# hasindu2008/slow5tools

Measured on AMD Instinct MI355X. Metric: blow5_encode_raw_signal_throughput, higher is better.
Workload: dtype int16->u8

## Files before the change

### slow5tools_amd/csrc/deflate2_dev.h

```cpp
#pragma once

namespace s5 {

__device__ __forceinline__ uint32_t alignbit(uint32_t hi, uint32_t lo, uint32_t sh) { return __builtin_amdgcn_alignbit(hi, lo, sh); }
__device__ __forceinline__ uint32_t zbytes(uint32_t x) {
    const uint32_t t = (x & 0x7F7F7F7Fu) + 0x7F7F7F7Fu;
    return ~(t | x | 0x7F7F7F7Fu);
}
__device__ __forceinline__ uint32_t frame_mask(int a0, int first, int len) {
    const int lo = min(4, max(0, first - a0)), hi = min(4, max(0, len - a0));
    const uint32_t mh = hi >= 4 ? 0xFFFFFFFFu : (1u << (8 * hi)) - 1u;
    const uint32_t ml = lo >= 4 ? 0xFFFFFFFFu : (1u << (8 * lo)) - 1u;
    return mh & ~ml & 0x80808080u;
}
__device__ __forceinline__ int top_slot(uint32_t m) { return (31 - __clz((int)m)) >> 3; }

__device__ __forceinline__ void length_symbol(int L, uint32_t &sym, uint32_t &eb, uint32_t &ev) {
    const int l = L - 3;
    eb = 0; ev = 0;
    if (L == 258) sym = 285;
    else if (l < 8) sym = 257 + l;
    else {
        const int nb = 29 - __clz(l);
        sym = 261 + 4 * nb + ((l >> nb) & 3);
// ... 49 lines not shown
struct SlabTail {
    uint32_t ql;
    uint32_t nfull;
    uint32_t rem;
    uint32_t runbyte;
};
struct WaveCarry {
    int lastb;
    bool ok;
};
__device__ __forceinline__ SlabTail slab_tail(const uint8_t *__restrict__ buf, int k, const SlabCls &c, WaveCarry &wc) {
    const int lane = lane_id();
    const int p0 = 256 * k + 4 * lane - 2;
    const uint32_t lastmem = c.member & ~c.Cp1;
    const uint32_t Bm = c.V & ~c.C;
    const int lb = Bm ? p0 + top_slot(Bm) : -1;
    const int Lincl = wave_incl_max(lb);
    const int Lprev = (int)wave_prev((uint32_t)Lincl, 0xFFFFFFFFu);
    const int slab_last = __builtin_amdgcn_readlane(Lincl, 63);
    SlabTail t;
    t.ql = 4; t.nfull = 0; t.rem = 0; t.runbyte = 0;
    int s = 0;
    const bool has = lastmem != 0u;
    if (has) {
        t.ql = (uint32_t)top_slot(lastmem);
        const uint32_t below = Bm & ((1u << (8 * t.ql)) - 1u);
        s = below ? p0 + top_slot(below) : Lprev;
    }
    if (__ballot(has && s < 0)) {
        if (!wc.ok) { wc.lastb = find_break_before(buf, 256 * k - 2); wc.ok = true; }
        if (has && s < 0) s = wc.lastb;
    }
    if (slab_last >= 0) { wc.lastb = slab_last; wc.ok = true; }
    if (has) {
        const int body = p0 + (int)t.ql - s;
        t.nfull = (uint32_t)((body * 16257) >> 22);
        t.rem = (uint32_t)body - 258u * t.nfull;
        t.runbyte = (c.bytes >> (8 * t.ql)) & 255u;
    }
    return t;
}

__device__ __forceinline__ uint32_t length_extra_bits(uint32_t sym) { return sym >= 265u && sym < 285u ? (sym - 261u) >> 2 : 0u; }
__device__ __forceinline__ uint32_t carry_e_before(const uint32_t *__restrict__ buf32, int k, int len) {
    const int di = 64 * k - 1;
    const uint32_t w = buf32[di], wp = buf32[di - 1];
    return (uint32_t)__builtin_amdgcn_readfirstlane((int)(zbytes(w ^ alignbit(w, wp, 24)) & frame_mask(4 * di, 1, len)));
}

constexpr uint32_t DEFL2_LIST_CAP = 640;
constexpr uint32_t DEFL2_LISTB_MIN = 64;
constexpr uint32_t SEG_FAST = 0xFFFFFFFFu, SEG_REDO = 0xFFFFFFFEu, SEG_MASK = 0xFFFFFFFDu;

template <int TN = NT>
__device__ __forceinline__ void deflate2_prepare(DeflShared &S, uint32_t *obuf, uint32_t obuf_words) {
    constexpr int NWV = TN / 64;
    typedef uint32_t u4a __attribute__((ext_vector_type(4)));
    u4a *w16 = reinterpret_cast<u4a *>(obuf + (obuf_words - (uint32_t)(NWV * 288)));
    for (int i = threadIdx.x; i < NWV * 72; i += TN) w16[i] = u4a{0u, 0u, 0u, 0u};
    if (threadIdx.x == 0) { S.lalloc = 0; S.red[7] = 0; }
}

template <int MODE, int TN = NT>
__device__ __forceinline__ void deflate_block2(DeflShared &S, uint32_t *obuf, uint32_t obuf_words, const uint8_t *__restrict__ buf, int len,
                                               bool final, ZOut &z, uint32_t &adA, uint32_t &adB, uint32_t dbg = 0,
                                               EarlySize es = EarlySize{nullptr, 0}, uint32_t gen_hint = 0, bool prepared = false) {
    static_assert(MODE == 1 || MODE == 2, "fused single block (1) or staged multi-block (2): the bit buffer is this function's to clear");
    constexpr bool FUSED = MODE == 1;
    constexpr int NWV = TN / 64;
    static_assert(TN % 64 == 0 && NWV >= 4 && NWV <= 8, "S.wtot holds four words per wave");
    const int tid = threadIdx.x, lane = lane_id();
    const int wv = __builtin_amdgcn_readfirstlane(wave_id());
    if (len == 0) {
        for (uint32_t i = tid; i < obuf_words; i += TN) obuf[i] = 0;
        __syncthreads();
        if (tid == 0) { if (FUSED) put_bits(obuf, z, 64, 0x9c78u, 16); else obuf[0] = z.carry; }
        if (tid == 0) put_bits(obuf, z, z.bitpos, (final ? 1u : 0u) | (1u << 1), 10);
        z.bitpos += 10;
        publish_size(es, z.bitpos);
        __syncthreads();
        return;
    }
    const uint32_t wf_at = obuf_words - (uint32_t)(NWV * 288);
    uint32_t *wfa = obuf + wf_at;
    uint32_t *wf = wfa + wv * 288;
    if (!prepared) {
        deflate2_prepare<TN>(S, obuf, obuf_words);
        __syncthreads();
    }

    const uint32_t *buf32 = reinterpret_cast<const uint32_t *>(buf);
    constexpr bool POOLB = MODE == 2;
    const bool poolb_ok = POOLB && wf_at >= DEFL2_LISTB_MIN + 64u;
    uint16_t *tla = reinterpret_cast<uint16_t *>(S.freq);
    uint16_t *tlb_top = reinterpret_cast<uint16_t *>(obuf + wf_at);
    const uint32_t list_cap = DEFL2_LIST_CAP + (poolb_ok ? (wf_at - DEFL2_LISTB_MIN) * 2u : 0u);
    const int nsl = (len + 2 + 255) >> 8;
#ifndef S5_DEFL2_GEN_W
#define S5_DEFL2_GEN_W 4
#endif
#ifndef S5_DEFL2_GEN_W_FUSED
#define S5_DEFL2_GEN_W_FUSED 5
#endif
    constexpr int GW = FUSED ? S5_DEFL2_GEN_W_FUSED : S5_DEFL2_GEN_W;
    const int gs = min(nsl, gen_hint ? (int)((gen_hint + 2u + 255u) >> 8) : 0);
    const int cost_all = (GW - 1) * gs + nsl;
    auto bound = [&](int w) -> int {
        if (w >= NWV) return nsl;
        const int T = (cost_all * w + NWV / 2) / NWV;
        return T <= GW * gs ? (T + GW / 2) / GW : gs + (T - GW * gs);
    };
    const int k0 = bound(wv), k1 = bound(wv + 1);
    uint32_t segs = SEG_FAST;

    {
        uint32_t a_acc = 0, b_acc = 0, d_acc = 0, nmatch = 0, nextra = 0;
        uint32_t carryE = k0 > 0 && k0 < k1 ? carry_e_before(buf32, k0, len) : 0u;
        WaveCarry wc{-1, k0 == 0};
        for (int k = k0; k < k1; k++) {
#ifndef S5_DEFL2_NO_PAIRS
            if (k >= gs && k > 0 && k + 1 < k1 && 256 * k + 512 <= len) {
                const int d0 = 64 * k + 2 * lane;
                const uint32_t wp = buf32[d0 - 1], w0 = buf32[d0], w1 = buf32[d0 + 1];
                const uint32_t E0 = zbytes(w0 ^ alignbit(w0, wp, 24)), E1 = zbytes(w1 ^ alignbit(w1, w0, 24));
                const uint32_t EpA = dpp_u32<DPP_WAVE_SHR1>(carryE, E1);
                auto member_of = [](uint32_t E, uint32_t Ep) {
                    const uint32_t C = alignbit(E, Ep, 16), Cm1 = alignbit(E, Ep, 8), Cp1 = alignbit(E, Ep, 24);
                    return C & ((Cp1 & (E | Cm1)) | (Ep & Cm1));
                };
                if (__ballot((member_of(E0, EpA) | member_of(E1, E0)) != 0u) == 0ull) {
                    carryE = (uint32_t)__builtin_amdgcn_readlane((int)E1, 63);
                    const uint32_t bA = alignbit(w0, wp, 16), bB = alignbit(w1, w0, 16);
                    atomicAdd(&wf[bA & 255u], 1u);
                    atomicAdd(&wf[(bA >> 8) & 255u], 1u);
                    atomicAdd(&wf[(bA >> 16) & 255u], 1u);
                    atomicAdd(&wf[bA >> 24], 1u);
                    atomicAdd(&wf[bB & 255u], 1u);
                    atomicAdd(&wf[(bB >> 8) & 255u], 1u);
                    atomicAdd(&wf[(bB >> 16) & 255u], 1u);
                    atomicAdd(&wf[bB >> 24], 1u);
                    const uint32_t wA = (uint32_t)(len - (256 * k + 8 * lane - 2));
                    const uint32_t sA = __builtin_amdgcn_udot4(bA, 0x01010101u, 0u, false), sB = __builtin_amdgcn_udot4(bB, 0x01010101u, 0u, false);
                    a_acc += sA + sB;
                    b_acc = __umul24(wA, sA) + __umul24(wA - 4u, sB) + b_acc;
                    d_acc = __builtin_amdgcn_udot4(bA, 0x03020100u, d_acc, false);
                    d_acc = __builtin_amdgcn_udot4(bB, 0x03020100u, d_acc, false);
                    wc.ok = false;
                    k++;
                    continue;
                }
            }
#endif
            const bool full = k > 0 && 256 * k + 256 <= len;
            const uint32_t wgt = (uint32_t)(len - (256 * k + 4 * lane - 2));
            SlabCls c;
            if (full) c = classify_slab<false>(buf32, k, len, carryE);
            else c = classify_slab<true>(buf32, k, len, carryE);
            const bool anymem = __ballot(c.member != 0u) != 0ull;
            if (full && !anymem) {
                atomicAdd(&wf[c.bytes & 255u], 1u);
                atomicAdd(&wf[(c.bytes >> 8) & 255u], 1u);
                atomicAdd(&wf[(c.bytes >> 16) & 255u], 1u);
                atomicAdd(&wf[c.bytes >> 24], 1u);
                const uint32_t s4 = __builtin_amdgcn_udot4(c.bytes, 0x01010101u, 0u, false);
                a_acc += s4;
                b_acc = __umul24(wgt, s4) + b_acc;
                d_acc = __builtin_amdgcn_udot4(c.bytes, 0x03020100u, d_acc, false);
                wc.ok = false;
                continue;
            }
            {
                uint32_t bytes = c.bytes;
// ... 373 lines not shown
```

### slow5tools_amd/csrc/deflate_dev.h

```cpp
#pragma once
#include "dev_common.h"

namespace s5 {

constexpr int DEFL_BLK = NT * 64;
constexpr int NLIT = 286;
constexpr int DOFF = 288;

template <int CAP>
struct BuildScratchT {
    alignas(16) uint32_t lf[CAP];
    alignas(16) uint32_t nf[CAP];
    uint16_t npar[CAP];
    uint16_t rsym[CAP];
};
struct SortScratch {
    uint32_t bm[64 * 9];
    uint32_t cnt[64];
    uint32_t ovl[288];
};
struct BuildScratch : BuildScratchT<288> { SortScratch sort; };

struct DeflShared {
    alignas(16) uint32_t freq[320];
// ... 419 lines not shown
    {
        static constexpr uint32_t CLA[19] = {0x30001, 0x7002f, 0x7006f, 0x7001f, 0x7005f, 0x50003, 0x50013, 0x5000b, 0x5001b, 0x50007,
                                             0x30005, 0x20000, 0x20002, 0x7003f, 0x00000, 0x00000, 0x50017, 0x6000f, 0x7007f};
        static constexpr uint32_t CLB[19] = {0x30002, 0x60017, 0x7002f, 0x7006f, 0x60037, 0x5000b, 0x40005, 0x5001b, 0x50007, 0x4000d,
                                             0x30006, 0x30001, 0x20000, 0x7001f, 0x7005f, 0x7003f, 0x40003, 0x6000f, 0x7007f};
        const uint32_t ca = lane < 19 ? CLA[lane] : 0u, cb = lane < 19 ? CLB[lane] : 0u;
        const uint32_t f = lane < 19 ? S.clfreq[lane] : 0u;
        const uint32_t eb = lane == 16 ? 2u : lane == 17 ? 3u : lane == 18 ? 7u : 0u;
        const uint32_t costA = wave_sum(f * ((ca >> 16) + eb) + ((f && !(ca >> 16)) ? (1u << 24) : 0u));
        const uint32_t costB = wave_sum(f * ((cb >> 16) + eb));
        const bool useA = costA <= costB;
        if (lane < 19) { const uint32_t c = useA ? ca : cb; S.clcode[lane] = c; S.cllens[lane] = (uint8_t)(c >> 16); }
        if (lane == 0) { S.red[6] = useA ? costA : costB; S.hclen = useA ? 18u : 19u; }
    }
}

template <int TN = NT>
__device__ __forceinline__ void flush_words(uint32_t *obuf, uint32_t *out32, ZOut &z, bool final_all, uint32_t n_words = 0xFFFFFFFFu) {
    const int tid = threadIdx.x;
    const uint32_t full = final_all ? (z.bitpos + 31) >> 5 : z.bitpos >> 5;
    const uint32_t n = n_words != 0xFFFFFFFFu ? n_words : full - z.flushed;
    {
        typedef uint32_t u4u __attribute__((ext_vector_type(4), aligned(4)));
        typedef uint32_t u4a __attribute__((ext_vector_type(4)));
        const u4a *s16 = reinterpret_cast<const u4a *>(obuf);
        const uint32_t nv = n >> 2;
        for (uint32_t j = tid; j < nv; j += TN) {
            const uint32_t w = z.flushed + 4u * j;
            const u4a v = s16[j];
            if (w >= 2) *reinterpret_cast<u4u *>(out32 + w) = v;
            else { out32[w + 2] = v.z; out32[w + 3] = v.w; }
        }
        for (uint32_t i = 4u * nv + tid; i < n; i += TN) {
            const uint32_t w = z.flushed + i;
            if (w >= 2) out32[w] = obuf[i];
        }
    }
    if (final_all) return;
    __syncthreads();
    const uint32_t partial = obuf[n];
    __syncthreads();
    for (uint32_t i = tid; i <= n; i += TN) obuf[i] = i == 0 ? partial : 0u;
    __syncthreads();
    z.flushed = full;
}

}
#include "deflate2_dev.h"
namespace s5 {

template <typename M>
__device__ __forceinline__ uint32_t zlib_frame_fused(DeflShared &S, uint32_t *obuf, uint32_t obuf_words, const uint8_t *pay,
                                                     uint32_t plen, ZOut &z, uint32_t dbg = 0, EarlySize es = EarlySize{nullptr, 0}, uint32_t gen_hint = 0,
                                                     bool prepared = false) {
    const int tid = threadIdx.x;
    z.bitpos = 80;
    z.flushed = 0;
    uint32_t adA = 1, adB = 0;
    deflate_block2<1, NT>(S, obuf, obuf_words, pay, (int)plen, true, z, adA, adB, dbg, es, gen_hint, prepared);
    if (dbg) return 16;
    z.bitpos = (z.bitpos + 7) & ~7u;
    if (tid == 0 && plen) {
        uint32_t a = 0, b = 0;
        for (int w = 0; w < NW; w++) { a += S.wad[w]; b += S.wad[8 + w]; }
        adB = (uint32_t)(((uint64_t)plen + b) % 65521u);
        adA = (1u + a) % 65521u;
    }
    if (tid == 0) put_bits(obuf, z, z.bitpos, __builtin_bswap32((adB << 16) | adA), 32);
    z.bitpos += 32;
    __syncthreads();
    return z.bitpos >> 3;
}

template <typename M>
__device__ __forceinline__ uint32_t zlib_compress_fused(DeflShared &S, uint32_t *obuf, uint32_t obuf_words,
                                                        const uint8_t *pay, uint32_t plen, uint8_t *out, uint32_t dbg = 0, uint32_t gen_hint = 0, bool prepared = false) {
    ZOut z;
    const uint32_t total = zlib_frame_fused<M>(S, obuf, obuf_words, pay, plen, z, dbg, EarlySize{nullptr, 0}, gen_hint, prepared);
    if (dbg) {
        if (threadIdx.x == 0) *reinterpret_cast<uint32_t *>(out) = z.bitpos;
        if (dbg == 41 && threadIdx.x < 20) reinterpret_cast<uint32_t *>(out)[4 + threadIdx.x] = threadIdx.x < 19 ? S.clfreq[threadIdx.x] : S.red[6];
        return 16;
    }
    flush_words(obuf, reinterpret_cast<uint32_t *>(out), z, true);
    if (threadIdx.x == 0) *reinterpret_cast<uint64_t *>(out) = (uint64_t)(total - 8);
    return total;
}

constexpr uint64_t LB_MASK = (1ull << 62) - 1;
__device__ __forceinline__ uint64_t wave_sum64(uint64_t v) {
#pragma unroll
    for (int d = 32; d >= 1; d >>= 1) v += __shfl_xor(v, d);
    return v;
}
template <int E = 1>
__device__ __forceinline__ uint64_t lookback_offset(unsigned long long *st, uint32_t r, uint64_t mysize, uint32_t *err, bool published) {
    const int lane = lane_id();
    if (!published && lane == 0) __hip_atomic_store(&st[r], (1ull << 62) | mysize, __ATOMIC_RELAXED, __HIP_MEMORY_SCOPE_AGENT);
    uint64_t acc = 0;
    long long base = (long long)r - 1;
    uint32_t spins = 0;
    for (;;) {
        uint64_t v[E];
#pragma unroll
        for (int e = 0; e < E; e++) {
            const long long idx = base - 64 * e - lane;
            v[e] = idx >= 0 ? __hip_atomic_load(&st[idx], __ATOMIC_RELAXED, __HIP_MEMORY_SCOPE_AGENT) : (2ull << 62);
        }
        int outcome = 0;
#pragma unroll
        for (int e = 0; e < E; e++) {
            if (outcome) continue;
            const uint32_t f = (uint32_t)(v[e] >> 62);
            const uint64_t m0 = __ballot(f == 0), m2 = __ballot(f == 2);
            const int first0 = m0 ? __ffsll((long long)m0) - 1 : 64;
            const int first2 = m2 ? __ffsll((long long)m2) - 1 : 64;
            if (first2 < first0) {
                acc += lane <= first2 ? (v[e] & LB_MASK) : 0ull;
                outcome = 1;
            } else {
                acc += lane < first0 ? (v[e] & LB_MASK) : 0ull;
                if (first0 < 64) { base -= 64 * e + first0; outcome = 2; }
            }
        }
        if (outcome == 1) break;
        if (outcome == 0) { base -= 64 * E; continue; }
        if (++spins > (1u << 22)) { if (lane == 0) *err = 1; break; }
        __builtin_amdgcn_s_sleep(2);
    }
    const uint64_t excl = wave_sum64(acc);
    if (lane == 0) __hip_atomic_store(&st[r], (2ull << 62) | (excl + mysize), __ATOMIC_RELAXED, __HIP_MEMORY_SCOPE_AGENT);
// ... 16 lines not shown
```

### slow5tools_amd/csrc/kernels.hip

```cpp
#include <hip/hip_runtime.h>
#include <limits.h>
#include <stdint.h>
#include <stdio.h>
#include <stdlib.h>
#include <string.h>

#include <atomic>
#include <mutex>
#include <type_traits>
#include <vector>

#include "../../include/slow5gpu.h"
#include "deflate_dev.h"
#include "lz_dev.h"
#include "inflate_dev.h"
#include "inflate_simt_dev.h"
#include "inflate_par_dev.h"
#include "zstd_dev.h"
#include "zstd_enc_dev.h"
#include "svb_dev.h"
#include "exzd_dev.h"
#include "order_dev.h"
#include "event_dev.h"
#include "enc_plan.h"

using namespace s5;

extern "C" void s5gpu_set_error(const char *fmt, ...);
int s5host_set_option(const char *key, long value);
namespace fsk { int set_option(const char *key, long value); }
namespace dfk { int set_option(const char *key, long value); }
namespace dtwk { int path_set_option(const char *key, long value); }
namespace pilek { int set_option(const char *key, long value); }
extern uint32_t s5host_generation;
static_assert(s5plan::BLK == (uint32_t)DEFL_BLK && s5plan::SIG_SVB_ZD == S5GPU_SIG_SVB_ZD && s5plan::SIG_EX_ZD == S5GPU_SIG_EX_ZD, "enc_plan.h restates these");

#define HIP_TRY(x)                                                                                   \
    do {                                                                                             \
        hipError_t e_ = (x);                                                                         \
        if (e_ != hipSuccess) {                                                                      \
            s5gpu_set_error("%s failed: %s (%s:%d)", #x, hipGetErrorString(e_), __FILE__, __LINE__); \
            return S5GPU_ERR_HIP;                                                                    \
        }                                                                                            \
    } while (0)

extern __shared__ __attribute__((aligned(16))) uint8_t smem[];

constexpr uint32_t S_BYTES = (sizeof(DeflShared) + 15u) & ~15u;
constexpr uint32_t BZ_BYTES = (sizeof(BuildScratch) + 15u) & ~15u;
constexpr uint32_t B_BYTES = NW * 288u * 4u + 64u;
constexpr uint32_t OVF = 0xFFFFFFFFu;

struct EncParams {
    s5gpu_encode_args_t a;
    uint32_t obuf_words;
    uint32_t pay_cap;
    uint32_t dbg;
    uint32_t zseq;
    uint32_t tier = 0;
};

static uint32_t g_fused_tier2 = 0;
static uint32_t g_zstd_sequences = 1;

__device__ __forceinline__ uint32_t payload_bound_dev(const s5gpu_read_desc_t &d, int sig_method) {
    const uint32_t n = d.n_samples;
    const uint32_t sig = sig_method == S5GPU_SIG_SVB_ZD ? 4 + ((n + 3) >> 2) + 3 * n
                       : sig_method == S5GPU_SIG_EX_ZD ? 24 + 2 * (((n + 3) >> 2) + 4 * n) + n : 2 * n;
    return d.hdr_len + 8 + sig + d.aux_len;
}

template <bool EXZD = false>
__device__ __forceinline__ uint32_t build_payload(const s5gpu_encode_args_t &a, const s5gpu_read_desc_t &d,
                                                  uint8_t *pay, uint32_t cap, uint32_t *ws, uint32_t *red = nullptr) {
    const int tid = threadIdx.x;
    const uint32_t n = d.n_samples;
    if constexpr (EXZD) {
        const uint32_t fixed_x = d.hdr_len + 8 + d.aux_len;
        if (fixed_x + 16 > cap) return OVF;
        const uint8_t *hdr = a.hdr + d.hdr_off;
        for (uint32_t i = tid; i < d.hdr_len; i += NT) pay[i] = hdr[i];
        uint8_t *lenp = pay + d.hdr_len;
        const uint32_t blen = exzd_encode_wg(a.sig + d.sig_off, n, lenp + 8, ws, red, cap - fixed_x);
        if (blen == EXZD_ERR) return OVF;
        if (tid < 8) lenp[tid] = tid < 4 ? (uint8_t)(blen >> (8 * tid)) : 0;
        if (d.aux_len) {
            const uint8_t *aux = a.aux + d.aux_off;
            uint8_t *ap = lenp + 8 + blen;
            for (uint32_t i = tid; i < d.aux_len; i += NT) ap[i] = aux[i];
        }
        return d.hdr_len + 8 + blen + d.aux_len;
    } else {
    const bool svb = a.sig_method == S5GPU_SIG_SVB_ZD;
    const uint32_t nk = (n + 3) >> 2;
    const uint32_t fixed = d.hdr_len + 8 + (svb ? 4 + nk : 0) + d.aux_len;
    if (fixed > cap || (svb ? n : 2 * n) > cap - fixed) return OVF;
    const uint8_t *hdr = a.hdr + d.hdr_off;
    for (uint32_t i = tid; i < d.hdr_len; i += NT) pay[i] = hdr[i];
    uint8_t *lenp = pay + d.hdr_len;
    uint8_t *sigp = lenp + 8;
    const int16_t *sig = a.sig + d.sig_off;
    uint64_t L;
    uint32_t sig_bytes;
    if (svb) {
        uint8_t *keys = sigp + 4;
        uint8_t *data = keys + nk;
        uint32_t total = 0;
        const uint32_t room = cap - fixed;
        for (uint32_t t0 = 0; t0 < n; t0 += SVB_TILE) {
            const uint32_t t = svb_encode_tile(sig, n, t0, keys + (t0 >> 2), data + total, ws, room - total, true);
            if (t > room - total) return OVF;
            total += t;
        }
        L = 4ull + nk + total;
        sig_bytes = (uint32_t)L;
// ... 33 lines not shown
        const uint32_t t = svb_encode_tile(sig, n, t0, reinterpret_cast<uint8_t *>(tile_keys), reinterpret_cast<uint8_t *>(tile_data), ws, OVF - 1);
        __syncthreads();
        const uint32_t tk = (min(n - t0, (uint32_t)SVB_TILE) + 3) >> 2;
        copy_record_out(tile_keys, tk, keys + (t0 >> 2));
        copy_record_out(tile_data, t, data + total);
        total += t;
        __syncthreads();
    }
    const uint64_t L = 4ull + nk + total;
    if (tid < 4) sigp[tid] = (uint8_t)(n >> (8 * tid));
    if (tid < 8) lenp[tid] = (uint8_t)(L >> (8 * tid));
    if (d.aux_len) {
        const uint8_t *aux = a.aux + d.aux_off;
        uint8_t *ap = sigp + (uint32_t)L;
        for (uint32_t i = tid; i < d.aux_len; i += NT) ap[i] = aux[i];
    }
    return d.hdr_len + 8 + (uint32_t)L + d.aux_len;
}

__device__ __forceinline__ uint32_t run_heavy_front(const s5gpu_encode_args_t &a, const s5gpu_read_desc_t &d) {
    return a.sig_method == S5GPU_SIG_SVB_ZD ? d.hdr_len + 12u + ((d.n_samples + 3u) >> 2) : 0u;
}

#ifndef S5_FUSED_HINT
#define S5_FUSED_HINT(a, d) run_heavy_front(a, d)
#endif

#ifndef S5_FUSED_WG_PER_CU
#define S5_FUSED_WG_PER_CU 8
#endif
template <typename M, bool EXZD = false, int WPS = S5_FUSED_WG_PER_CU>
__global__ __launch_bounds__(NT, WPS) void k_encode_fused(EncParams p) {
    const uint32_t r = blockIdx.x;
    if (p.tier == 2 && p.a.out_len[r] != 0) return;
    DeflShared &S = *reinterpret_cast<DeflShared *>(smem);
    uint32_t *obuf = reinterpret_cast<uint32_t *>(smem + S_BYTES);
    uint8_t *pay = smem + S_BYTES + 4u * p.obuf_words;
    const s5gpu_read_desc_t d = p.a.desc[r];
    deflate2_prepare<NT>(S, obuf, p.obuf_words);
    const uint32_t plen = build_payload<EXZD>(p.a, d, pay, p.pay_cap, S.ws, S.red);
    if (plen == OVF) {
        if (threadIdx.x == 0 && p.tier != 1) {
            const uint32_t at = atomicAdd(&p.a.ovf[0], 1u);
            p.a.ovf[1 + at] = r;
        }
        return;
    }
    __syncthreads();
    if (p.dbg == 1) {
        if (threadIdx.x == 0) p.a.out_len[r] = plen + pay[plen - 1];
        return;
    }
    uint8_t *out = p.a.slots + d.out_off;
    const uint32_t total = zlib_compress_fused<M>(S, obuf, p.obuf_words, pay, plen, out, p.dbg, S5_FUSED_HINT(p.a, d), true);
    if (threadIdx.x == 0) p.a.out_len[r] = total;
}

#ifndef S5_LB_E
#define S5_LB_E 1
#endif
struct StreamParams {
    unsigned long long *state;
    uint32_t *ctl;
    uint8_t *stream;
    uint64_t *rec_off;
};
template <typename M, bool EXZD = false>
__global__ __launch_bounds__(NT, S5_FUSED_WG_PER_CU) void k_encode_stream(EncParams p, StreamParams sp) {
    __shared__ uint32_t s_r;
    __shared__ uint64_t s_off;
    DeflShared &S = *reinterpret_cast<DeflShared *>(smem);
    uint32_t *obuf = reinterpret_cast<uint32_t *>(smem + S_BYTES);
    uint8_t *pay = smem + S_BYTES + 4u * p.obuf_words;
#ifdef S5_ES_NOTICKET
    const uint32_t r = blockIdx.x;
#else
    if (threadIdx.x == 0) s_r = atomicAdd(&sp.ctl[1], 1u);
    __syncthreads();
    const uint32_t r = s_r;
#endif
    const s5gpu_read_desc_t d = p.a.desc[r];
    deflate2_prepare<NT>(S, obuf, p.obuf_words);
    const uint32_t plen = build_payload<EXZD>(p.a, d, pay, p.pay_cap, S.ws, S.red);
    uint32_t total = 0;
    if (plen == OVF) {
        if (threadIdx.x == 0) atomicAdd(&sp.ctl[0], 1u);
    } else {
        __syncthreads();
        ZOut z;
        total = zlib_frame_fused<M>(S, obuf, p.obuf_words, pay, plen, z, 0, EarlySize{sp.state, r}, S5_FUSED_HINT(p.a, d), true);
        if (threadIdx.x == 0) { obuf[0] = total - 8; obuf[1] = 0; }
    }
    if (wave_id() == 0) {
        const uint64_t off = lookback_offset<S5_LB_E>(sp.state, r, total, &sp.ctl[2], plen != OVF);
        if (lane_id() == 0) {
            s_off = off;
            sp.rec_off[r] = off;
            if (r == p.a.n_reads - 1) sp.rec_off[p.a.n_reads] = off + total;
            p.a.out_len[r] = total;
        }
    }
    __syncthreads();
    if (total) copy_record_out(obuf, total, sp.stream + s_off);
}

__device__ __forceinline__ uint32_t park_offset(const s5gpu_read_desc_t &d, int sig_method) {
    return (d.slot_cap - payload_bound_dev(d, sig_method)) & ~15u;
}

#ifndef S5_PACK_WG
#define S5_PACK_WG 8
#endif
__global__ __launch_bounds__(NT, S5_PACK_WG) void k_pack(EncParams p, int mode, const uint32_t *ord) {
    __shared__ uint32_t ws[16];
    __shared__ __attribute__((aligned(16))) uint32_t tile_keys[SVB_TILE / 16 + 4];
    __shared__ __attribute__((aligned(16))) uint32_t tile_data[3 * SVB_TILE / 4 + 4];
    const uint32_t count = mode == 2 ? p.a.ovf[0] : p.a.n_reads;
    for (uint32_t it = blockIdx.x; it < count; it += gridDim.x) {
        const uint32_t r = mode == 2 ? ovf_at(p.a.ovf, ord, it) : it;
        const s5gpu_read_desc_t d = p.a.desc[r];
        uint8_t *dst = p.a.slots + d.out_off + (mode == 1 ? 8u : park_offset(d, p.a.sig_method));
        const uint32_t plen = build_payload_hbm(p.a, d, dst, ws, tile_keys, tile_data);
        if (threadIdx.x == 0) {
            if (mode == 1) {
                *reinterpret_cast<uint64_t *>(p.a.slots + d.out_off) = plen;
                p.a.out_len[r] = plen + 8;
            } else {
                p.a.out_len[r] = plen;
            }
        }
        __syncthreads();
    }
}

#ifndef S5_STAGED_TN
#define S5_STAGED_TN 256
#endif
struct StagedPf { uint4 v[DEFL_BLK / 16 / S5_STAGED_TN]; };
__device__ __forceinline__ void staged_fetch(StagedPf &pf, const uint8_t *src, uint32_t at, uint32_t plen) {
    const uint32_t bl = min(plen - at, (uint32_t)DEFL_BLK);
    const uint4 *s4 = reinterpret_cast<const uint4 *>(src + at);
#pragma unroll
    for (int j = 0; j < DEFL_BLK / 16 / S5_STAGED_TN; j++) {
        const uint32_t i = threadIdx.x + j * S5_STAGED_TN;
        pf.v[j] = i < (bl + 15) / 16 ? s4[i] : uint4{0u, 0u, 0u, 0u};
    }
}
__device__ __forceinline__ uint32_t deflate_staged_record(const EncParams &p, uint32_t r, const s5gpu_read_desc_t &d, uint32_t plen, DeflShared &S, uint32_t *obuf, BuildScratch &B, uint8_t *stage,
                                                          StagedPf &pf, const uint8_t *next_src, uint32_t next_plen) {
    const int tid = threadIdx.x;
    uint8_t *out = p.a.slots + d.out_off;
    const uint8_t *src = out + park_offset(d, p.a.sig_method);
// ... 1180 lines not shown
template <class Key>
static int build_order(const Key &key, uint32_t n, bool list, uint32_t long_bucket, hipStream_t st, const uint32_t **out,
                       std::unique_lock<std::mutex> &hold, size_t extra_words = 0, uint32_t **extra = nullptr) {
    *out = nullptr;
    if (extra) *extra = nullptr;
    if (!list && !(extra && extra_words)) return S5GPU_OK;
    const size_t list_words = list ? (((size_t)ORD_LIST + n + 3) & ~(size_t)3) : 0;
    uint32_t *p = nullptr;
    { const int rc = order_scratch(st, list_words + (extra ? extra_words : 0), &p, hold); if (rc) return rc; }
    if (!p) return S5GPU_OK;
    if (list) {
        const uint32_t nb = (n + NT - 1) / NT;
        hipLaunchKernelGGL(k_order_zero, dim3(1), dim3(NT), 0, st, p);
        hipLaunchKernelGGL(k_order_count<Key>, dim3(nb), dim3(NT), 0, st, key, p);
        hipLaunchKernelGGL(k_order_scan, dim3(1), dim3(128), 0, st, p, long_bucket);
        hipLaunchKernelGGL(k_order_scatter<Key>, dim3(nb), dim3(NT), 0, st, key, p);
        *out = p;
    }
    if (extra && extra_words) *extra = p + list_words;
    return S5GPU_OK;
}
static int launch_order(const s5gpu_decode_args_t *a, hipStream_t st, const uint32_t **out, std::unique_lock<std::mutex> &hold,
                        size_t extra_words = 0, uint32_t **extra = nullptr, bool want_order = true) {
    const bool order = want_order && g_order_min && a->n_recs >= g_order_min;
    return build_order(OrderByInLen{a->desc, a->n_recs}, a->n_recs, order, 0, st, out, hold, extra_words, extra);
}
static uint32_t g_zstd_pre_min = 256;
static size_t zstd_pre_words(const s5gpu_decode_args_t *a) {
    return g_zstd_pre_min && a->n_recs >= g_zstd_pre_min ? (size_t)a->n_recs * (ZW_REC / 4) : 0;
}
static int launch_eorder(const s5gpu_encode_args_t *a, hipStream_t st, const uint32_t **out, std::unique_lock<std::mutex> &hold) {
    const bool order = g_order_min && a->n_reads >= g_order_min;
    return build_order(OrderOvfBySamples{a->desc, a->ovf}, a->n_reads, order, 0, st, out, hold);
}
int s5kern_digest_order(const digk::DigRecs &R, hipStream_t st, const uint32_t **out, std::unique_lock<std::mutex> &hold) {
    return build_order(OrderByCanonLen{R.desc, R.fields, R.n}, R.n, R.n > 16, 0, st, out, hold);
}
int s5kern_event_order(const sigk::SigRecs &R, hipStream_t st, const uint32_t **out, std::unique_lock<std::mutex> &hold) {
    return build_order(OrderBySigLen{R}, R.n, R.n > 64, 0, st, out, hold);
}

static bool rec_method_ok(int m) { return m == S5GPU_REC_NONE || m == S5GPU_REC_ZLIB || m == S5GPU_REC_ZSTD; }
static bool sig_method_ok(int m) { return m == S5GPU_SIG_NONE || m == S5GPU_SIG_SVB_ZD || m == S5GPU_SIG_EX_ZD; }
static int enc_check(const s5gpu_encode_args_t *a) {
    if (!a || (a->n_reads && (!a->desc || !a->sig || !a->hdr || !a->slots || !a->out_len))) return S5GPU_ERR_ARG;
    return rec_method_ok(a->rec_method) && sig_method_ok(a->sig_method) ? S5GPU_OK : S5GPU_ERR_ARG;
}

static EncParams enc_params(const s5gpu_encode_args_t *a, bool dbg = false) {
    EncParams p;
    p.a = *a;
    p.dbg = dbg && getenv("S5GPU_DEBUG_STAGE") ? (uint32_t)atoi(getenv("S5GPU_DEBUG_STAGE")) : 0;
    p.zseq = g_zstd_sequences;
    p.obuf_words = 0; p.pay_cap = 0;
    return p;
}
static size_t staged_shape(EncParams &p) {
    p.obuf_words = (DEFL_BLK + 64) / 4; p.pay_cap = DEFL_BLK;
    return S_BYTES + 4ull * p.obuf_words + DEFL_BLK;
}
static size_t fused_shape(EncParams &p, uint32_t cap, uint32_t floor) {
    p.obuf_words = (cap + 64 > floor ? cap + 64 : floor) / 4; p.pay_cap = cap;
    return S_BYTES + 4ull * p.obuf_words + cap;
}
static int stream_params(StreamParams *sp, uint32_t n_reads, uint8_t *stream_out, uint64_t *rec_off, uint64_t *state, uint32_t *ctl, hipStream_t st) {
    *sp = StreamParams{reinterpret_cast<unsigned long long *>(state), ctl, stream_out, rec_off};
    HIP_TRY(hipMemsetAsync(state, 0, 8ull * n_reads, st));
    HIP_TRY(hipMemsetAsync(ctl, 0, 16, st));
    return S5GPU_OK;
}

using EncodeKernel = void (*)(EncParams);
using StreamKernel = void (*)(EncParams, StreamParams);
static const EncodeKernel ENCODE_FUSED[] = {k_encode_fused<uint32_t, false>, k_encode_fused<uint32_t, true>, k_encode_fused<uint64_t, false>, k_encode_fused<uint64_t, true>,
                                            k_encode_fused<uint64_t, false, 4>};
static const StreamKernel ENCODE_STREAM[] = {k_encode_stream<uint32_t, false>, k_encode_stream<uint32_t, true>, k_encode_stream<uint64_t, false>, k_encode_stream<uint64_t, true>};
static const EncodeKernel ZSTD_FUSED[] = {k_zstd_fused<false>, k_zstd_fused<true>};
static EncodeKernel encode_fused_kernel(bool wide, bool exzd, bool four_per_cu = false) { return ENCODE_FUSED[four_per_cu ? 4 : 2 * wide + exzd]; }
static StreamKernel encode_stream_kernel(bool wide, bool exzd) { return ENCODE_STREAM[2 * wide + exzd]; }
static EncodeKernel zstd_fused_kernel(bool exzd) { return ZSTD_FUSED[exzd]; }
static const void *const LDS_KERNELS[] = {(const void *)k_deflate_staged, (const void *)k_deflate_lz<LzLong>, (const void *)k_deflate_lz<LzShort>, (const void *)k_zstd_staged,
                                          (const void *)k_svbzd_encode, (const void *)k_svbzd_stream, (const void *)k_inflate_simt<false>, (const void *)k_inflate_simt<true>};

constexpr int DEV_MAX = 64;
struct DeviceFacts {
    std::atomic<bool> attrs{false};
    std::atomic<int> cus{0};
    std::atomic<uint32_t> np_resident[6];
} static g_dev[DEV_MAX];
static DeviceFacts *device_facts() {
    int dev = -1;
    return hipGetDevice(&dev) == hipSuccess && dev >= 0 && dev < DEV_MAX ? &g_dev[dev] : nullptr;
}
static int device_cus(int *cus) {
    DeviceFacts *f = device_facts();
    *cus = f ? f->cus.load(std::memory_order_relaxed) : 0;
    if (*cus > 0) return S5GPU_OK;
    int dev = 0;
    HIP_TRY(hipGetDevice(&dev));
    HIP_TRY(hipDeviceGetAttribute(cus, hipDeviceAttributeMultiprocessorCount, dev));
    if (f && *cus > 0) f->cus.store(*cus, std::memory_order_relaxed);
    return S5GPU_OK;
}
static int set_lds_attrs() {
    DeviceFacts *f = device_facts();
    if (f && f->attrs.load(std::memory_order_acquire)) return S5GPU_OK;
// ... 94 lines not shown
        return S5GPU_ERR_ARG;
    }
    if (a->n_reads == 0) return S5GPU_OK;
    int rc;
    if ((rc = set_lds_attrs())) return rc;
    hipStream_t st = (hipStream_t)stream_;
    EncParams p = enc_params(a);
    StreamParams sp;
    if ((rc = stream_params(&sp, a->n_reads, stream_out, rec_off, state, ctl, st))) return rc;
    const uint32_t cap = s5plan::fused_cap(a->sig_method, a->max_payload, a->lds_payload_cap, DEFL_BLK);
    const size_t lds = fused_shape(p, cap, B_BYTES);
    hipLaunchKernelGGL(encode_stream_kernel(s5plan::wide(cap), a->sig_method == S5GPU_SIG_EX_ZD), dim3(a->n_reads), dim3(NT), lds, st, p, sp);
    HIP_TRY(hipGetLastError());
    return S5GPU_OK;
}

extern "C" int s5gpu_pack_parked_dev(const s5gpu_encode_args_t *a, void *stream_) {
    int rc = enc_check(a);
    if (rc) { s5gpu_set_error("s5gpu_pack_parked_dev: bad arguments"); return rc; }
    if (a->n_reads == 0) return S5GPU_OK;
    EncParams p = enc_params(a);
    staged_shape(p);
    hipLaunchKernelGGL(k_pack, dim3(a->n_reads), dim3(NT), 0, (hipStream_t)stream_, p, 0, nullptr);
    HIP_TRY(hipGetLastError());
    return S5GPU_OK;
}

extern "C" int s5gpu_deflate_parked_dev(const s5gpu_encode_args_t *a, void *stream_) {
    int rc = enc_check(a);
    if (rc) { s5gpu_set_error("s5gpu_deflate_parked_dev: bad arguments"); return rc; }
    if (a->n_reads == 0) return S5GPU_OK;
    if ((rc = set_lds_attrs())) return rc;
    EncParams p = enc_params(a);
    const size_t lds = staged_shape(p);
    if (a->rec_method == S5GPU_REC_ZSTD) hipLaunchKernelGGL(k_zstd_staged, dim3(a->n_reads), dim3(NT), lds, (hipStream_t)stream_, p, 0);
    else if (a->sig_method == S5GPU_SIG_NONE)
        launch_lz(p, a->n_reads, a->max_payload, (hipStream_t)stream_);
    else hipLaunchKernelGGL(k_deflate_staged, dim3(a->n_reads), dim3(S5_STAGED_TN), lds, (hipStream_t)stream_, p, 0, nullptr);
    HIP_TRY(hipGetLastError());
    return S5GPU_OK;
}

static uint32_t g_unpack_fused = 1;
static uint32_t g_inflate_par = 1;
static uint32_t g_inflate_route = 1;
static uint32_t g_np_lds_payload = 1;
static uint32_t g_inflate_simt_min = 24576;
static const struct Option { const char *name; uint32_t *var; long lo, hi; uint32_t keep; } OPTIONS[] = {
    {"inflate_simt_min", &g_inflate_simt_min, 0, LONG_MAX, ~0u},
    {"inflate_route", &g_inflate_route, 0, 1, ~0u},
    {"np_lds_payload", &g_np_lds_payload, 0, 1, ~0u},
    {"fused_tier2", &g_fused_tier2, 0, DEFL_BLK, ~15u},
    {"zstd_sequences", &g_zstd_sequences, 0, 1, ~0u},
    {"unpack_fused", &g_unpack_fused, 0, 1, ~0u},
    {"inflate_par", &g_inflate_par, 0, 2, ~0u},
    {"zstd_pre_min", &g_zstd_pre_min, 0, LONG_MAX, ~0u},
    {"order_min", &g_order_min, 0, LONG_MAX, ~0u},
};
extern "C" int s5gpu_set_option(const char *key, long value) {
    for (const Option &o : OPTIONS)
        if (key && strcmp(key, o.name) == 0 && value >= o.lo && value <= o.hi) { *o.var = (uint32_t)value & o.keep; return S5GPU_OK; }
    if (s5host_set_option(key, value) == S5GPU_OK || fsk::set_option(key, value) == S5GPU_OK || dfk::set_option(key, value) == S5GPU_OK ||
        dtwk::path_set_option(key, value) == S5GPU_OK || pilek::set_option(key, value) == S5GPU_OK)
        return S5GPU_OK;
    s5gpu_set_error("s5gpu_set_option: unknown option");
    return S5GPU_ERR_ARG;
}
struct AuxStream {
    hipStream_t st = nullptr;
    hipEvent_t fork = nullptr, join = nullptr;
    int dev = -1;
};
static std::mutex g_aux_mu;
static std::vector<AuxStream *> g_aux_all, g_aux_free;
static int aux_acquire(AuxStream **out) {
    int dev = 0;
    HIP_TRY(hipGetDevice(&dev));
    {
        std::lock_guard<std::mutex> lk(g_aux_mu);
        for (size_t i = 0; i < g_aux_free.size(); i++)
            if (g_aux_free[i]->dev == dev) { *out = g_aux_free[i]; g_aux_free.erase(g_aux_free.begin() + (long)i); return S5GPU_OK; }
    }
    AuxStream *a = new AuxStream();
    a->dev = dev;
    if (hipStreamCreateWithFlags(&a->st, hipStreamNonBlocking) != hipSuccess || hipEventCreateWithFlags(&a->fork, hipEventDisableTiming) != hipSuccess ||
        hipEventCreateWithFlags(&a->join, hipEventDisableTiming) != hipSuccess) {
        if (a->st) (void)hipStreamDestroy(a->st);
        if (a->fork) (void)hipEventDestroy(a->fork);
        delete a;
        s5gpu_set_error("helper stream for the routed inflate could not be created");
        return S5GPU_ERR_HIP;
    }
    std::lock_guard<std::mutex> lk(g_aux_mu);
    g_aux_all.push_back(a);
    *out = a;
    return S5GPU_OK;
}
static void aux_release(AuxStream *a, uint32_t gen) {
    std::lock_guard<std::mutex> lk(g_aux_mu);
    if (gen == s5host_generation) g_aux_free.push_back(a);
}
void s5kern_release_aux() {
    std::lock_guard<std::mutex> lk(g_aux_mu);
    for (AuxStream *a : g_aux_all) {
        (void)hipStreamDestroy(a->st);
        (void)hipEventDestroy(a->fork);
// ... 350 lines not shown
```

Baseline: 686.9.

## Add run-list front pass for the generated prefix of fused deflate blocks

Result: no change. 685.5 (-0.2%).

```diff
diff --git a/slow5tools_amd/csrc/deflate2_dev.h b/slow5tools_amd/csrc/deflate2_dev.h
--- a/slow5tools_amd/csrc/deflate2_dev.h
+++ b/slow5tools_amd/csrc/deflate2_dev.h
@@ -125,6 +125,107 @@
 constexpr uint32_t DEFL2_LISTB_MIN = 64;
 constexpr uint32_t SEG_FAST = 0xFFFFFFFFu, SEG_REDO = 0xFFFFFFFEu, SEG_MASK = 0xFFFFFFFDu;
 
+#ifndef S5_DEFL2_RUNS_PER_SLAB
+#define S5_DEFL2_RUNS_PER_SLAB 128
+#endif
+constexpr int DEFL2_RUNS_HW = S5_DEFL2_RUNS_PER_SLAB + 2;
+__device__ __forceinline__ bool front_runs(DeflShared &S, uint32_t *obuf, uint32_t *wf, const uint8_t *__restrict__ buf, int len, int ka, int kb,
+                                           uint32_t carryE, uint32_t &a_acc, uint32_t &b_acc, uint32_t &d_acc, uint32_t &nmatch, uint32_t &nextra,
+                                           uint32_t &segs) {
+    const int lane = lane_id();
+    const uint32_t *buf32 = reinterpret_cast<const uint32_t *>(buf);
+    const int R0 = ka ? 256 * ka - 2 : 0, R1 = 256 * kb - 2;
+    uint16_t *L = reinterpret_cast<uint16_t *>(obuf) + DEFL2_RUNS_HW * ka;
+    const uint32_t lcap = (uint32_t)(DEFL2_RUNS_HW * (kb - ka)) - 1u;
+    const int ent = ka > 0 ? __builtin_amdgcn_readfirstlane((int)(buf[R0] == buf[R0 - 1])) : 0;
+    int nbk = 0;
+    uint32_t aa = 0, bb = 0, dd = 0, ub = 0;
+    for (int k = ka; k < kb; k++) {
+        const bool full = k > 0 && 256 * k + 256 <= len;
+        SlabCls c;
+        if (full) c = classify_slab<false>(buf32, k, len, carryE);
+        else c = classify_slab<true>(buf32, k, len, carryE);
+        uint32_t bytes = c.bytes;
+        if (!full) { const uint32_t vb = c.V >> 7; bytes &= (vb << 8) - vb; }
+        const uint32_t s4 = __builtin_amdgcn_udot4(bytes, 0x01010101u, 0u, false);
+        aa += s4;
+        bb = __umul24((uint32_t)(len - (256 * k + 4 * lane - 2)), s4) + bb;
+        dd = __builtin_amdgcn_udot4(bytes, 0x03020100u, dd, false);
+        ub += (uint32_t)__popc(c.V & ~c.member) + 2u * (uint32_t)__popc(c.member & ~c.Cp1);
+        const uint32_t Bm = c.V & ~c.C;
+        const uint32_t pop = (uint32_t)__popc(Bm);
+        const uint32_t incl = wave_incl_add(pop);
+        uint32_t at = (uint32_t)(ent + nbk) + incl - pop;
+        const uint32_t p0 = (uint32_t)(256 * k + 4 * lane - 2);
+#pragma unroll
+        for (int q = 0; q < 4; q++)
+            if (Bm & (0x80u << (8 * q))) L[min(at++, lcap)] = (uint16_t)(p0 + q);
+        nbk += __builtin_amdgcn_readlane((int)incl, 63);
+    }
+    if (nbk > S5_DEFL2_RUNS_PER_SLAB * (kb - ka)) return false;
+    const int nr = nbk + ent;
+    int sE = R0;
+    {
+        const int p = R1 + lane;
+        const bool brk = lane >= 3 || p >= len || buf[p] != buf[p - 1];
+        const int qend = R1 + __ffsll((long long)__ballot(brk)) - 1;
+        if (ent) sE = find_break_before(buf, R0);
+        if (lane == 0) { L[nr] = (uint16_t)qend; if (ent) L[0] = (uint16_t)sE; }
+    }
+    wave_sync();
+    const uint32_t room = wave_sum(ub) + (uint32_t)(((R1 - sE) * 16257) >> 22);
+    uint32_t st = 0;
+    if (lane == 0) st = atomicAdd(&S.lalloc, room);
+    st = (uint32_t)__builtin_amdgcn_readfirstlane((int)st);
+    const bool listed = st + room <= DEFL2_LIST_CAP;
+    uint16_t *tl = reinterpret_cast<uint16_t *>(S.freq);
+    uint32_t base = st;
+    for (int j0 = 0; j0 < nr; j0 += 64) {
+        const int j = j0 + lane;
+        int s = 0;
+        uint32_t own = 0, nfull = 0, mlen = 0, nl = 0;
+        if (j < nr) {
+            s = L[j];
+            const int q = L[j + 1];
+            own = s >= R0 ? 1u : 0u;
+            const int body = q - s - 1;
+            if (body < 3) nl = (uint32_t)max(0, min(q, R1) - max(s + 1, R0));
+            else if (q <= R1) {
+                nfull = (uint32_t)((body * 16257) >> 22);
+                const uint32_t rem = (uint32_t)body - 258u * nfull;
+                if (rem >= 3u) mlen = rem; else nl = rem;
+            }
+        }
+        const uint32_t ext = nfull + (mlen ? 1u : nl), cnt = own + ext;
+        const uint32_t incl = wave_incl_add(cnt);
+        if (cnt) {
+            const uint32_t b = buf[s];
+            uint32_t at = base + incl - cnt;
+            uint32_t last = b;
+            if (own + nl) atomicAdd(&wf[b], own + nl);
+            if (nfull) atomicAdd(&wf[285], nfull);
+            if (mlen) {
+                uint32_t tsym, teb, tev;
+                length_symbol((int)mlen, tsym, teb, tev);
+                atomicAdd(&wf[tsym], 1u);
+                nextra += teb;
+                last = tsym | (tev << 9);
+            }
+            nmatch += nfull + (mlen ? 1u : 0u);
+            if (listed) {
+                if (own) tl[at] = (uint16_t)b;
+                at += own;
+#pragma unroll 1
+                for (uint32_t i = 0; i < ext; i++) tl[at + i] = (uint16_t)(i < nfull ? 285u : last);
+            }
+        }
+        base += (uint32_t)__builtin_amdgcn_readlane((int)incl, 63);
+    }
+    if (lane < kb - ka) segs = listed ? st | (lane == 0 ? (base - st) << 16 : 0u) : SEG_REDO;
+    a_acc += aa; b_acc += bb; d_acc += dd;
+    return true;
+}
+
 template <int TN = NT>
 __device__ __forceinline__ void deflate2_prepare(DeflShared &S, uint32_t *obuf, uint32_t obuf_words) {
     constexpr int NWV = TN / 64;
@@ -137,7 +238,8 @@
 template <int MODE, int TN = NT>
 __device__ __forceinline__ void deflate_block2(DeflShared &S, uint32_t *obuf, uint32_t obuf_words, const uint8_t *__restrict__ buf, int len,
                                                bool final, ZOut &z, uint32_t &adA, uint32_t &adB, uint32_t dbg = 0,
-                                               EarlySize es = EarlySize{nullptr, 0}, uint32_t gen_hint = 0, bool prepared = false) {
+                                               EarlySize es = EarlySize{nullptr, 0}, uint32_t gen_hint = 0, bool prepared = false,
+                                               bool front = true) {
     static_assert(MODE == 1 || MODE == 2, "fused single block (1) or staged multi-block (2): the bit buffer is this function's to clear");
     constexpr bool FUSED = MODE == 1;
     constexpr int NWV = TN / 64;
@@ -190,7 +292,16 @@
         uint32_t a_acc = 0, b_acc = 0, d_acc = 0, nmatch = 0, nextra = 0;
         uint32_t carryE = k0 > 0 && k0 < k1 ? carry_e_before(buf32, k0, len) : 0u;
         WaveCarry wc{-1, k0 == 0};
-        for (int k = k0; k < k1; k++) {
+        int kfirst = k0;
+        if (FUSED && front) {
+            const int kb = min(k1, (int)(min(gen_hint, (uint32_t)len) + 2u) >> 8);
+            if (kb > k0 && (uint32_t)(DEFL2_RUNS_HW * kb + 1) / 2u <= wf_at && front_runs(S, obuf, wf, buf, len, k0, kb, carryE, a_acc, b_acc, d_acc, nmatch, nextra, segs)) {
+                kfirst = kb;
+                if (kb < k1) carryE = carry_e_before(buf32, kb, len);
+                wc = WaveCarry{-1, false};
+            }
+        }
+        for (int k = kfirst; k < k1; k++) {
 #ifndef S5_DEFL2_NO_PAIRS
             if (k >= gs && k > 0 && k + 1 < k1 && 256 * k + 512 <= len) {
                 const int d0 = 64 * k + 2 * lane;
diff --git a/slow5tools_amd/csrc/deflate_dev.h b/slow5tools_amd/csrc/deflate_dev.h
--- a/slow5tools_amd/csrc/deflate_dev.h
+++ b/slow5tools_amd/csrc/deflate_dev.h
@@ -495,12 +495,12 @@
 template <typename M>
 __device__ __forceinline__ uint32_t zlib_frame_fused(DeflShared &S, uint32_t *obuf, uint32_t obuf_words, const uint8_t *pay,
                                                      uint32_t plen, ZOut &z, uint32_t dbg = 0, EarlySize es = EarlySize{nullptr, 0}, uint32_t gen_hint = 0,
-                                                     bool prepared = false) {
+                                                     bool prepared = false, bool front_runs = true) {
     const int tid = threadIdx.x;
     z.bitpos = 80;
     z.flushed = 0;
     uint32_t adA = 1, adB = 0;
-    deflate_block2<1, NT>(S, obuf, obuf_words, pay, (int)plen, true, z, adA, adB, dbg, es, gen_hint, prepared);
+    deflate_block2<1, NT>(S, obuf, obuf_words, pay, (int)plen, true, z, adA, adB, dbg, es, gen_hint, prepared, front_runs);
     if (dbg) return 16;
     z.bitpos = (z.bitpos + 7) & ~7u;
     if (tid == 0 && plen) {
@@ -517,9 +517,10 @@
 
 template <typename M>
 __device__ __forceinline__ uint32_t zlib_compress_fused(DeflShared &S, uint32_t *obuf, uint32_t obuf_words,
-                                                        const uint8_t *pay, uint32_t plen, uint8_t *out, uint32_t dbg = 0, uint32_t gen_hint = 0, bool prepared = false) {
+                                                        const uint8_t *pay, uint32_t plen, uint8_t *out, uint32_t dbg = 0, uint32_t gen_hint = 0, bool prepared = false,
+                                                        bool front_runs = true) {
     ZOut z;
-    const uint32_t total = zlib_frame_fused<M>(S, obuf, obuf_words, pay, plen, z, dbg, EarlySize{nullptr, 0}, gen_hint, prepared);
+    const uint32_t total = zlib_frame_fused<M>(S, obuf, obuf_words, pay, plen, z, dbg, EarlySize{nullptr, 0}, gen_hint, prepared, front_runs);
     if (dbg) {
         if (threadIdx.x == 0) *reinterpret_cast<uint32_t *>(out) = z.bitpos;
         if (dbg == 41 && threadIdx.x < 20) reinterpret_cast<uint32_t *>(out)[4 + threadIdx.x] = threadIdx.x < 19 ? S.clfreq[threadIdx.x] : S.red[6];
diff --git a/slow5tools_amd/csrc/kernels.hip b/slow5tools_amd/csrc/kernels.hip
--- a/slow5tools_amd/csrc/kernels.hip
+++ b/slow5tools_amd/csrc/kernels.hip
@@ -57,10 +57,12 @@
     uint32_t pay_cap;
     uint32_t dbg;
     uint32_t zseq;
+    uint32_t front_runs;
     uint32_t tier = 0;
 };
 
 static uint32_t g_fused_tier2 = 0;
+static uint32_t g_front_runs = 1;
 static uint32_t g_zstd_sequences = 1;
 
 __device__ __forceinline__ uint32_t payload_bound_dev(const s5gpu_read_desc_t &d, int sig_method) {
@@ -200,8 +202,12 @@
         return;
     }
     uint8_t *out = p.a.slots + d.out_off;
-    const uint32_t total = zlib_compress_fused<M>(S, obuf, p.obuf_words, pay, plen, out, p.dbg, S5_FUSED_HINT(p.a, d), true);
+    const uint32_t total = zlib_compress_fused<M>(S, obuf, p.obuf_words, pay, plen, out, p.dbg, S5_FUSED_HINT(p.a, d), true, p.front_runs != 0);
+#ifdef S5_DEFL2_CHECK
+    if (threadIdx.x == 0) p.a.out_len[r] = total | (S.red[7] ? 0x80000000u : 0u);
+#else
     if (threadIdx.x == 0) p.a.out_len[r] = total;
+#endif
 }
 
 #ifndef S5_LB_E
@@ -236,7 +242,7 @@
     } else {
         __syncthreads();
         ZOut z;
-        total = zlib_frame_fused<M>(S, obuf, p.obuf_words, pay, plen, z, 0, EarlySize{sp.state, r}, S5_FUSED_HINT(p.a, d), true);
+        total = zlib_frame_fused<M>(S, obuf, p.obuf_words, pay, plen, z, 0, EarlySize{sp.state, r}, S5_FUSED_HINT(p.a, d), true, p.front_runs != 0);
         if (threadIdx.x == 0) { obuf[0] = total - 8; obuf[1] = 0; }
     }
     if (wave_id() == 0) {
@@ -245,7 +251,11 @@
             s_off = off;
             sp.rec_off[r] = off;
             if (r == p.a.n_reads - 1) sp.rec_off[p.a.n_reads] = off + total;
+#ifdef S5_DEFL2_CHECK
+            p.a.out_len[r] = total | (S.red[7] ? 0x80000000u : 0u);
+#else
             p.a.out_len[r] = total;
+#endif
         }
     }
     __syncthreads();
@@ -1532,6 +1542,7 @@
     p.a = *a;
     p.dbg = dbg && getenv("S5GPU_DEBUG_STAGE") ? (uint32_t)atoi(getenv("S5GPU_DEBUG_STAGE")) : 0;
     p.zseq = g_zstd_sequences;
+    p.front_runs = g_front_runs;
     p.obuf_words = 0; p.pay_cap = 0;
     return p;
 }
@@ -1732,6 +1743,7 @@
     {"np_lds_payload", &g_np_lds_payload, 0, 1, ~0u},
     {"fused_tier2", &g_fused_tier2, 0, DEFL_BLK, ~15u},
     {"zstd_sequences", &g_zstd_sequences, 0, 1, ~0u},
+    {"front_runs", &g_front_runs, 0, 1, ~0u},
     {"unpack_fused", &g_unpack_fused, 0, 1, ~0u},
     {"inflate_par", &g_inflate_par, 0, 2, ~0u},
     {"zstd_pre_min", &g_zstd_pre_min, 0, LONG_MAX, ~0u},
```
